# Idokorro/MiniGrid-RL

Measured on AMD Instinct MI355X. Metric: env-steps/sec at 65k parallel envs, 1/2/4/8 MI355X; % HBM roofline, higher is better.
Workload: dtype u8

## Files before the change

### minigrid-rl_amd/csrc/mgx_device.h

```cpp
#pragma once
#ifndef MGX_HOST_SIM
#include <hip/hip_runtime.h>
#else
#include "host_sim.h"
#endif
#include <stdint.h>

#include "mgx_diag.h"

namespace mgx {

constexpr uint8_t CODE_EMPTY = 0x01;
constexpr uint8_t CODE_WALL = 2 | (5 << 4);
constexpr uint8_t CODE_GOAL = 8 | (1 << 4);
constexpr uint8_t CODE_LAVA = 9;
constexpr int T_EMPTY = 1, T_WALL = 2, T_DOOR = 4, T_KEY = 5, T_BALL = 6, T_BOX = 7,
              T_GOAL = 8, T_LAVA = 9, T_OPEN = 11;
constexpr int A_LEFT = 0, A_RIGHT = 1, A_FORWARD = 2, A_PICKUP = 3, A_DROP = 4,
              A_TOGGLE = 5, A_DONE = 6;
constexpr uint8_t NONE8 = 0xFF;

__device__ __forceinline__ int cn2idx(int cn) { return (0x403512 >> (cn * 4)) & 0xF; }

__device__ __forceinline__ uint8_t mk_code(int t, int cidx, int aux) {
// ... 121 lines not shown
        x = (int)(a >> k);
        y = (int)(b >> k);
        return;
    }
    const uint64_t ma = (uint64_t)a * s, mb = (uint64_t)b * s;
    if ((uint32_t)ma < s || (uint32_t)mb < s) {
        p = p0;
        x = pcg_integers(p, 0, S);
        y = pcg_integers(p, 0, S);
        return;
    }
    x = (int)(ma >> 32);
    y = (int)(mb >> 32);
}

__device__ __forceinline__ uint32_t ss_hashmix(uint32_t v, uint32_t &hc) {
    v ^= hc; hc *= 0x931e8875u; v *= hc; v ^= v >> 16; return v;
}
__device__ __forceinline__ uint32_t ss_mix(uint32_t x, uint32_t y) {
    uint32_t r = 0xca01f9ddu * x - 0x4973f715u * y; r ^= r >> 16; return r;
}
__device__ __forceinline__ void pcg_seed(Pcg &p, uint64_t seed) {
    uint32_t e0 = (uint32_t)seed, e1 = (uint32_t)(seed >> 32);
    int nent = (seed >> 32) ? 2 : 1;
    uint32_t pool[4];
    uint32_t hc = 0x43b0d7e5u;
#pragma unroll
    for (int i = 0; i < 4; i++) pool[i] = ss_hashmix(i == 0 ? e0 : (i == 1 && nent == 2 ? e1 : 0u), hc);
#pragma unroll
    for (int s = 0; s < 4; s++)
#pragma unroll
        for (int d = 0; d < 4; d++)
            if (s != d) pool[d] = ss_mix(pool[d], ss_hashmix(pool[s], hc));
    uint32_t w[8];
    uint32_t hb = 0x8b51f9ddu;
#pragma unroll
    for (int i = 0; i < 8; i++) {
        uint32_t v = pool[i & 3];
        v ^= hb; hb *= 0x58f38dedu; v *= hb; v ^= v >> 16;
        w[i] = v;
    }
    uint64_t v0 = (uint64_t)w[0] | ((uint64_t)w[1] << 32), v1 = (uint64_t)w[2] | ((uint64_t)w[3] << 32);
    uint64_t v2 = (uint64_t)w[4] | ((uint64_t)w[5] << 32), v3 = (uint64_t)w[6] | ((uint64_t)w[7] << 32);
    p.ih = (v2 << 1) | (v3 >> 63);
    p.il = (v3 << 1) | 1ull;
    p.sh = 0; p.sl = 0;
    pcg_step(p);
    uint64_t nl = p.sl + v1;
    p.sh = p.sh + v0 + (nl < p.sl ? 1ull : 0ull);
    p.sl = nl;
    pcg_step(p);
    p.has = 0; p.uinteger = 0;
}

constexpr int MT_FIELDS = 10;
template <int NW>
__host__ __device__ constexpr int mt_wg() { return NW == 1 ? MGX_MT_WG1 : 16; }
constexpr int MT_WG_MAX = 16;
template <int NW>
__host__ __device__ constexpr int win_stride() { return 2 * mt_wg<NW>() + 2; }
__host__ __device__ constexpr int win_stride_of(int nw) { return nw == 1 ? win_stride<1>() : win_stride<2>(); }
constexpr uint64_t MT_REP = 0x041041041041041ull;
constexpr uint64_t MT_LOW60 = (1ull << 60) - 1ull;
constexpr int MAX_OBJS = 32;
constexpr int SAT_PROBE = 64;
constexpr uint32_t PCG_LOOP_LIMIT = 1u << 20;

template <int NW>
struct Bits {
    uint64_t w0, w1, w2, w3;
    __device__ __forceinline__ void clear() { w0 = w1 = w2 = w3 = 0; }
    __device__ __forceinline__ bool test(int b) const {
        const int i = b >> 6;
        uint64_t v = w0;
        if (NW > 1) v = i == 1 ? w1 : v;
        if (NW > 2) { v = i == 2 ? w2 : v; v = i == 3 ? w3 : v; }
        return (v >> (b & 63)) & 1ull;
    }
    __device__ __forceinline__ void set(int b) {
        const int i = b >> 6;
        const uint64_t m = 1ull << (b & 63);
        w0 |= i == 0 ? m : 0ull;
        if (NW > 1) w1 |= i == 1 ? m : 0ull;
        if (NW > 2) { w2 |= i == 2 ? m : 0ull; w3 |= i == 3 ? m : 0ull; }
    }
    __device__ __forceinline__ void unset(int b) {
        const int i = b >> 6;
        const uint64_t m = ~(1ull << (b & 63));
        w0 &= i == 0 ? m : ~0ull;
        if (NW > 1) w1 &= i == 1 ? m : ~0ull;
        if (NW > 2) { w2 &= i == 2 ? m : ~0ull; w3 &= i == 3 ? m : ~0ull; }
    }
};

template <>
struct Bits<4> {
    __device__ __forceinline__ void clear() {}
    __device__ __forceinline__ void set(int) {}
    __device__ __forceinline__ void unset(int) {}
};

template <int NW>
struct Gen {
    uint8_t *g;
    int S;
    Bits<NW> occ;
    Bits<NW> dn;
    const uint64_t *table;
    uint64_t rmask;
    uint64_t tlo, thi;
    uint64_t *win;
    uint64_t gbase;
    uint64_t cur, astart;
    uint64_t ga, gb, gc;
    uint64_t gi;
    int go;
    uint32_t llw;
    bool abort;
    uint32_t err;
    Pcg pcg;
    int ax, ay, adir;
    int goalx, goaly;
    bool phave;
    uint64_t prec;
    uint32_t *objs;
    int nobjs;
    uint32_t tmask;
    int problem, cfg_mission, num_objects, all_doors_open, n_obstacles;
#if MGX_GEN_STAMPS
    unsigned long long *stamps;
    uint64_t tlast;
#endif
};

#if MGX_GEN_STAMPS
#define GSTAMP(G, k)                                                                     \
    do {                                                                                 \
        const uint64_t _t = __builtin_amdgcn_s_memtime();                                \
        const unsigned long long _m = __ballot(1);                                       \
        if ((int)__lane_id() == __ffsll((long long)_m) - 1) atomicAdd(&(G).stamps[k], _t - (G).tlast); \
        (G).tlast = _t;                                                                  \
    } while (0)
#if MGX_GEN_STAMPS == 2
#define GCOUNT(G, k) do { } while (0)
#else
#define GCOUNT(G, k)                                                                     \
    do {                                                                                 \
        const unsigned long long _m = __ballot(1);                                       \
        if ((int)__lane_id() == __ffsll((long long)_m) - 1) atomicAdd(&(G).stamps[k], 1ull); \
    } while (0)
#endif
#else
#define GSTAMP(G, k) do { } while (0)
#define GCOUNT(G, k) do { } while (0)
#endif


template <int NW>
__device__ __forceinline__ void put(Gen<NW> &G, int x, int y, uint8_t code) {
    const int b = y * G.S + x;
    G.g[b] = code;
    if (code == CODE_EMPTY) G.occ.unset(b); else G.occ.set(b);
}

#ifndef MGX_HOST_SIM
typedef __attribute__((address_space(3))) uint64_t lds_u64;
#else
typedef uint64_t lds_u64;
#endif
constexpr int MT_PAD = MT_WG_MAX + 4;
template <int WG>
__device__ __noinline__ void mt_refill_cold(const uint64_t *__restrict__ table, uint64_t slot, lds_u64 *win) {
    const uint4 *src = reinterpret_cast<const uint4 *>(table + slot);
    static_assert(WG % 8 == 0 && WG <= MT_WG_MAX, "window loads go in fours of 16 B");
#pragma unroll
    for (int h = 0; h < WG / 8; h++) {
        const uint4 v0 = src[4 * h], v1 = src[4 * h + 1], v2 = src[4 * h + 2], v3 = src[4 * h + 3];
        lds_u64 *d = win + 8 * h;
        d[0] = (uint64_t)v0.x | ((uint64_t)v0.y << 32); d[1] = (uint64_t)v0.z | ((uint64_t)v0.w << 32);
        d[2] = (uint64_t)v1.x | ((uint64_t)v1.y << 32); d[3] = (uint64_t)v1.z | ((uint64_t)v1.w << 32);
        d[4] = (uint64_t)v2.x | ((uint64_t)v2.y << 32); d[5] = (uint64_t)v2.z | ((uint64_t)v2.w << 32);
        d[6] = (uint64_t)v3.x | ((uint64_t)v3.y << 32); d[7] = (uint64_t)v3.z | ((uint64_t)v3.w << 32);
    }
}
template <int NW>
__device__ __forceinline__ uint64_t win_group(Gen<NW> &G, uint64_t g) {
    constexpr int MT_WG = mt_wg<NW>();
    uint64_t off = g - G.gbase;
    if (off >= MT_WG) {
        GCOUNT(G, 23);
        if (g < G.tlo || g + MT_WG > G.thi) G.err |= 1u;
        mt_refill_cold<MT_WG>(G.table, g & G.rmask, (lds_u64 *)G.win);
        G.gbase = g;
        off = 0;
    }
    return G.win[off];
}
__device__ __forceinline__ uint64_t div10(uint64_t v) { return __umul64hi(v, 0xCCCCCCCCCCCCCCCDull) >> 3; }
template <int NW>
__device__ __forceinline__ void mt_sync(Gen<NW> &G) {
    const uint64_t g = div10(G.cur);
    G.go = (int)(G.cur - g * MT_FIELDS);
    G.gi = g;
    G.ga = win_group(G, g);
    G.gb = win_group(G, g + 1);
    G.gc = win_group(G, g + 2);
}
struct RbConst {
    uint64_t c1;
    uint32_t sh;
};
__device__ __forceinline__ RbConst rb_const(uint32_t n) {
    const uint32_t sh = 5u - (uint32_t)(32 - __clz(n));
    return RbConst{(uint64_t)(32u + (n << sh) - 1u) * MT_REP, sh};
}
template <int NW>
__device__ __forceinline__ int randbelow_c(Gen<NW> &G, const RbConst K);
template <int NW>
__device__ __forceinline__ int randbelow(Gen<NW> &G, uint32_t n) {
    GCOUNT(G, 24);
    if (n >= 32u) { G.err |= 8u; return 0; }
    return randbelow_c(G, rb_const(n));
}
template <int NW>
__device__ __forceinline__ int randbelow_c(Gen<NW> &G, const RbConst K) {
    const uint64_t c1 = K.c1;
    const uint32_t sh = K.sh;
    for (;;) {
        GCOUNT(G, 21);
        const int o6 = (int)__umul24((uint32_t)G.go, 6u);
        const uint64_t f = ((G.ga >> o6) | (G.gb << (60 - o6))) & MT_LOW60;
        const uint64_t acc = (c1 - f) & (32ull * MT_REP);
        const uint32_t left = G.llw - (uint32_t)(G.cur - G.astart);
        const int j = acc ? (int)(((uint32_t)__ffsll((long long)acc) - 1u - 5u) * 171u >> 10) : MT_FIELDS;
        int m = j < MT_FIELDS ? j + 1 : MT_FIELDS;
        if ((uint32_t)m > left) {
            G.cur = G.astart + G.llw;
            G.abort = true;
            return 0;
        }
        const int r = (int)(((f >> (6 * (j < MT_FIELDS ? j : 0))) & 31u) >> sh);
        G.cur += (uint64_t)m;
        G.go += m;
        if (G.go >= MT_FIELDS) {
            G.go -= MT_FIELDS;
            G.ga = G.gb;
            G.gb = G.gc;
            G.gi++;
            G.gc = win_group(G, G.gi + 2);
        }
        if (j < MT_FIELDS) return r;
    }
}
template <class GT>
__device__ __forceinline__ void mt_advance(GT &G, int m) {
    G.cur += (uint64_t)m;
    G.go += m;
    if (G.go >= MT_FIELDS) {
        G.go -= MT_FIELDS;
        G.ga = G.gb;
        G.gb = G.gc;
        G.gi++;
        G.gc = win_group(G, G.gi + 2);
    }
}
template <class GT>
__device__ __forceinline__ uint64_t randbelow_seq(GT &G, uint64_t prog, int cnt) {
    constexpr uint64_t GM = 32ull * MT_REP;
    uint64_t res = 0;
    int i = 0;
#pragma unroll 1
    while (i < cnt) {
        GCOUNT(G, 21);
        const int o6 = (int)__umul24((uint32_t)G.go, 6u);
        const uint64_t f = ((G.ga >> o6) | (G.gb << (60 - o6))) & MT_LOW60;
        uint64_t avail = GM;
        int used = MT_FIELDS;
#pragma unroll 1
        while (i < cnt) {
            const RbConst K = rb_const((uint32_t)(prog >> (5 * i)) & 31u);
            const uint64_t acc = (K.c1 - f) & avail;
            if (!acc) { used = MT_FIELDS; break; }
            const int b = __ffsll((long long)acc) - 1;
            res |= (uint64_t)((((uint32_t)(f >> (b - 5))) & 31u) >> K.sh) << (5 * i);
            avail &= ~((2ull << b) - 1ull);
            used = (int)((uint32_t)(b + 1) * 171u >> 10);
            i++;
        }
        const uint32_t left = G.llw - (uint32_t)(G.cur - G.astart);
        if ((uint32_t)used > left) {
            G.cur = G.astart + G.llw;
            G.abort = true;
            return res;
        }
        mt_advance(G, used);
    }
    return res;
}
template <int NW, typename Bad, typename Sat>
__device__ __forceinline__ void draw_cell(Gen<NW> &G, const RbConst KX, const RbConst KY, int x0, int y0, int &x, int &y,
                                          Bad bad, Sat sat ,
                                          bool has_c, const RbConst KC, int &choice) {
    constexpr uint64_t GM = 32ull * MT_REP;
    int rej = 0;
    bool need_c = has_c;
#pragma unroll 1
    for (;;) {
        GCOUNT(G, 21);
        const int o6 = (int)__umul24((uint32_t)G.go, 6u);
        const uint64_t f = ((G.ga >> o6) | (G.gb << (60 - o6))) & MT_LOW60;
        uint64_t avail = GM;
        int used = 0;
        if (need_c) {
            const uint64_t acc = (KC.c1 - f) & GM;
            if (!acc) {
                const uint32_t left = G.llw - (uint32_t)(G.cur - G.astart);
                if ((uint32_t)MT_FIELDS > left) {
                    G.cur = G.astart + G.llw;
                    G.abort = true;
                    return;
                }
                mt_advance(G, MT_FIELDS);
                continue;
            }
            const int b = __ffsll((long long)acc) - 1;
            choice = (int)((((uint32_t)(f >> (b - 5))) & 31u) >> KC.sh);
            avail &= ~((2ull << b) - 1ull);
            used = (int)((uint32_t)(b + 1) * 171u >> 10);
            need_c = false;
        }
        const uint64_t accx = (KX.c1 - f) & GM, accy = (KY.c1 - f) & GM;
        bool ok = false;
#pragma unroll 1
        for (;;) {
            const uint64_t cx = accx & avail;
            if (!cx) break;
            const int bx = __ffsll((long long)cx) - 1;
            const uint64_t cy = accy & avail & ~((2ull << bx) - 1ull);
            if (!cy) break;
            const int by = __ffsll((long long)cy) - 1;
            x = x0 + (int)(((uint32_t)(f >> (bx - 5)) & 31u) >> KX.sh);
            y = y0 + (int)(((uint32_t)(f >> (by - 5)) & 31u) >> KY.sh);
            used = (int)((uint32_t)(by + 1) * 171u >> 10);
            avail &= ~((2ull << by) - 1ull);
            if (!bad(x, y)) { ok = true; break; }
            if (++rej == SAT_PROBE && !sat()) { live_lock(G); return; }
        }
        const uint32_t left = G.llw - (uint32_t)(G.cur - G.astart);
        if ((uint32_t)used > left) {
            G.cur = G.astart + G.llw;
            G.abort = true;
            return;
        }
        mt_advance(G, used);
        if (ok) return;
        x = x0 + randbelow_c(G, KX);
        y = y0 + randbelow_c(G, KY);
        if (G.abort) return;
        if (!bad(x, y)) return;
        if (++rej == SAT_PROBE && !sat()) { live_lock(G); return; }
    }
}

template <int NW>
__device__ __forceinline__ int randint(Gen<NW> &G, int a, int b) { return a + randbelow(G, (uint32_t)(b - a + 1)); }
template <int NW>
__device__ __forceinline__ bool choice_bool(Gen<NW> &G) { return randbelow(G, 2) == 0; }

template <int NW>
__device__ __forceinline__ bool next2door(const Gen<NW> &G, int x, int y) {
    if constexpr (NW == 4) {
        return is_door(G.g[y * G.S + x - 1]) || is_door(G.g[y * G.S + x + 1]) ||
               is_door(G.g[(y - 1) * G.S + x]) || is_door(G.g[(y + 1) * G.S + x]);
    } else {
        return G.dn.test(y * G.S + x);
    }
}
template <int NW>
__device__ __forceinline__ bool occupied(const Gen<NW> &G, int b) {
    if constexpr (NW == 4) return G.g[b] != CODE_EMPTY;
    else return G.occ.test(b);
}

constexpr uint32_t OBJ_KEYFLAG = 1u << 24;
template <int NW>
__device__ __forceinline__ void add_obj(Gen<NW> &G, int t, int cname, int x, int y, uint32_t flags = 0) {
    const bool full = G.nobjs >= MAX_OBJS;
    G.err |= full ? 8u : 0u;
    G.tmask |= full ? 0u : 1u << t;
    const bool first_goal = !full && t == T_GOAL && G.goalx < 0;
    G.goalx = first_goal ? x : G.goalx;
    G.goaly = first_goal ? y : G.goaly;
    if (!full)
        G.objs[G.nobjs++] = (uint32_t)t | ((uint32_t)(cname & 15) << 4) | ((uint32_t)x << 8) | ((uint32_t)y << 16) | flags;
}

template <int NW>
__device__ __forceinline__ void draw_free_cell(Gen<NW> &G, int &px, int &py) {
    for (uint32_t it = 0;; ++it) {
        GCOUNT(G, 22);
        if (it > PCG_LOOP_LIMIT) { G.err |= 4u; px = 1; py = 1; return; }
        int x, y;
        pcg_cell(G.pcg, G.S, x, y);
        if (occupied(G, y * G.S + x)) continue;
        if (x == G.ax && y == G.ay) continue;
        px = x; py = y;
        return;
    }
}
template <int NW>
__device__ __forceinline__ void place_agent(Gen<NW> &G) {
    G.ax = -1; G.ay = -1;
    int x, y;
    draw_free_cell(G, x, y);
    G.ax = x; G.ay = y;
    G.adir = pcg_integers(G.pcg, 0, 4);
}

__device__ __forceinline__ int nth_set_bit(uint32_t m, int r) {
    int pos = 0, c;
    c = __popc(m & 0xFFFFu); if (r >= c) { r -= c; m >>= 16; pos += 16; }
    c = __popc(m & 0xFFu);   if (r >= c) { r -= c; m >>= 8;  pos += 8; }
    c = __popc(m & 0xFu);    if (r >= c) { r -= c; m >>= 4;  pos += 4; }
    c = __popc(m & 0x3u);    if (r >= c) { r -= c; m >>= 2;  pos += 2; }
    c = (int)(m & 1u);       if (r >= c) { pos += 1; }
    return pos;
}
template <int NW>
__device__ __forceinline__ int mask_choice(Gen<NW> &G, uint32_t m) {
    return nth_set_bit(m, randbelow(G, (uint32_t)__popc(m)));
}

template <int NW>
__device__ __forceinline__ void live_lock(Gen<NW> &G) {
    G.cur = G.astart + G.llw;
    G.abort = true;
}

template <int NW>
__device__ __forceinline__ void place_key(Gen<NW> &G, int x0, int x1, int y0, int y1, int gx, int gy, bool chk_agent,
                                          int ox, int oy, int cname, bool kib, int *kx, int *ky) {
    int x, y, rej = 0;
    for (;;) {
        x = randint(G, x0, x1);
        y = randint(G, y0, y1);
        if (G.abort) return;
        const bool bad = (x == gx && y == gy) || (chk_agent && x == G.ax && y == G.ay) || (x == ox && y == oy) ||
                         next2door(G, x, y);
        if (!bad) break;
        if (++rej == SAT_PROBE) {
            bool sat = false;
            for (int xx = x0; xx <= x1 && !sat; xx++)
                for (int yy = y0; yy <= y1 && !sat; yy++)
                    sat = !((xx == gx && yy == gy) || (chk_agent && xx == G.ax && yy == G.ay) ||
                            (xx == ox && yy == oy) || next2door(G, xx, yy));
            if (!sat) { live_lock(G); return; }
        }
    }
    const int cidx = cn2idx(cname);
    if (kib) { put(G, x, y, mk_code(T_BOX, cidx, 1)); add_obj(G, T_BOX, cname, x, y, OBJ_KEYFLAG); }
    else { put(G, x, y, mk_code(T_KEY, cidx, 0)); add_obj(G, T_KEY, cname, x, y, OBJ_KEYFLAG); }
    if (kx) { *kx = x; *ky = y; }
}

template <int NW>
__device__ __forceinline__ void place_objects(Gen<NW> &G, uint32_t &oc, const int *types, int n, int x0, int x1,
                                              int y0, int y1) {
    for (int k = 0; k < n; k++) {
        if (oc == 0) { G.err |= 8u; return; }
        const int b = mask_choice(G, oc);
        if (G.abort) return;
        oc &= ~(1u << b);
        const int t = types[b / 6], cname = b % 6;
        int x, y, rej = 0;
        for (;;) {
            x = randint(G, x0, x1);
            y = randint(G, y0, y1);
            if (G.abort) return;
            const bool bad = occupied(G, y * G.S + x) || (x == G.ax && y == G.ay) || next2door(G, x, y);
            if (!bad) break;
            if (++rej == SAT_PROBE) {
                bool sat = false;
                for (int xx = x0; xx <= x1 && !sat; xx++)
                    for (int yy = y0; yy <= y1 && !sat; yy++)
                        sat = !(occupied(G, yy * G.S + xx) || (xx == G.ax && yy == G.ay) || next2door(G, xx, yy));
                if (!sat) { live_lock(G); return; }
            }
        }
        put(G, x, y, mk_code(t, cn2idx(cname), 0));
        add_obj(G, t, cname, x, y);
    }
}

__device__ __forceinline__ int door_code(int cname, bool locked, bool open) {
    return open ? mk_code(T_OPEN, cn2idx(cname), 0) : mk_code(T_DOOR, cn2idx(cname), locked ? 1 : 0);
}

template <int NW>
__device__ __forceinline__ void put_door(Gen<NW> &G, int x, int y, uint8_t code) {
    put(G, x, y, code);
    const int S = G.S, b = y * S + x;
    if (x > 0) G.dn.set(b - 1);
    if (x < S - 1) G.dn.set(b + 1);
    if (y > 0) G.dn.set(b - S);
    if (y < S - 1) G.dn.set(b + S);
}

template <int NW>
__device__ __forceinline__ uint32_t bits_row(const Bits<NW> &B, int y, int S) {
    const int b = y * S;
    uint64_t v = b < 64 ? (B.w0 >> b) : 0ull;
    if (NW > 1) {
        if (b >= 64) v = B.w1 >> (b - 64);
// ... 67 lines not shown
    } else if (r == 1) {
        if (ar == 1) { kA = VL; kB = HL; } else if (ar == 3) kA = HL; else if (ar == 0) kA = VL;
    } else if (r == 2) {
        if (ar == 2) { kA = VU; kB = HR; } else if (ar == 3) kA = VU; else if (ar == 0) kA = HR;
    } else {
        if (ar == 3) { kA = VL; kB = HR; } else if (ar == 1) kA = HR; else if (ar == 2) kA = VL;
    }
}

__device__ const int MULTI_TYPES[3] = {T_KEY, T_BALL, T_BOX};

struct Prefix {
    int nr, rc;
    uint32_t dinfo;
    uint32_t dpos;
    uint32_t dopen;
};
template <class GT>
__device__ __forceinline__ void prefix_draws(GT &G, int S, bool draw_cmd, bool ado, Prefix &P) {
    const uint64_t r = randbelow_seq(G, draw_cmd ? (4ull | (3ull << 5)) : 3ull, draw_cmd ? 2 : 1);
    P.rc = draw_cmd ? (int)(r & 31) : 0;
    P.nr = 2 + (int)((draw_cmd ? r >> 5 : r) & 31);
    P.dinfo = P.dpos = P.dopen = 0;
    if (G.abort || (MGX_GEN_SKIP & 8)) return;
    const int nr = P.nr, mid = S / 2, ndoors = nr == 2 ? 1 : nr;
    uint64_t prog = 0;
    int cnt = 0;
#pragma unroll 1
    for (int d = 0; d < ndoors; d++) {
        prog |= (uint64_t)(6 - d) << (5 * cnt++);
        if (!ado) prog |= 2ull << (5 * cnt++);
        prog |= 2ull << (5 * cnt++);
    }
    const uint64_t dr = randbelow_seq(G, prog, cnt);
    if (G.abort) return;
    uint32_t dc = 0x3Fu;
#pragma unroll 1
    for (int d = 0, k = 0; d < ndoors; d++) {
        const int col = nth_set_bit(dc, (int)(dr >> (5 * k++)) & 31);
        dc &= ~(1u << col);
        const bool lk = ado ? false : ((dr >> (5 * k++)) & 31) == 0;
        const bool kib = ((dr >> (5 * k++)) & 31) == 0;
        P.dinfo |= (uint32_t)(col | (lk << 3) | (kib << 4)) << (8 * d);
    }
    prog = 0;
    cnt = 0;
#pragma unroll 1
    for (int d = 0; d < ndoors; d++) {
        bool horiz; int lo, hi;
        door_geom(nr, d, mid, S, horiz, lo, hi);
        prog |= (uint64_t)(hi - lo + 1) << (5 * cnt++);
        if (ado) prog |= 2ull << (5 * cnt++);
    }
    const uint64_t pr = randbelow_seq(G, prog, (MGX_GEN_SKIP & 2) ? 0 : cnt);
    if (G.abort) return;
#pragma unroll 1
    for (int d = 0, k = 0; d < ((MGX_GEN_SKIP & 2) ? 0 : ndoors); d++) {
        P.dpos |= (uint32_t)((pr >> (5 * k++)) & 15) << (4 * d);
        if (ado) P.dopen |= (uint32_t)(((pr >> (5 * k++)) & 31) == 0) << d;
    }
}
constexpr int PFX_LOOK = 320;
__host__ __device__ __forceinline__ uint64_t pfx_pack(const Prefix &P, uint32_t adv, uint32_t tag) {
    uint64_t r = (uint64_t)(adv & 0xFF) | ((uint64_t)(tag & 0xFF) << 8) | ((uint64_t)(P.nr - 2) << 16) |
                 ((uint64_t)(P.rc & 3) << 18);
    for (int d = 0; d < 4; d++)
        r |= (uint64_t)(((P.dinfo >> (8 * d)) & 31) | (((P.dpos >> (4 * d)) & 15) << 5) | (((P.dopen >> d) & 1) << 9))
             << (20 + 10 * d);
    return r;
}
__host__ __device__ __forceinline__ void pfx_unpack(uint64_t r, Prefix &P) {
    P.nr = 2 + (int)((r >> 16) & 3);
    P.rc = (int)((r >> 18) & 3);
    P.dinfo = P.dpos = P.dopen = 0;
    for (int d = 0; d < 4; d++) {
        const uint32_t f = (uint32_t)(r >> (20 + 10 * d)) & 0x3FFu;
        P.dinfo |= (f & 31u) << (8 * d);
        P.dpos |= ((f >> 5) & 15u) << (4 * d);
        P.dopen |= ((f >> 9) & 1u) << d;
    }
}
constexpr int MT_SB_WORDS = 3120;
constexpr int MT_SB_GROUPS = MT_SB_WORDS / MT_FIELDS;
constexpr int MT_SLIDE_MAX_SB = 64;
__host__ __device__ __forceinline__ int mt_slide_superblocks(unsigned long long hi, unsigned long long need_lo,
                                                             unsigned long long want_hi,
                                                             unsigned long long ring_groups) {
    int nsb = 0;
    while (nsb < MT_SLIDE_MAX_SB && hi + (unsigned long long)nsb * MT_SB_GROUPS < want_hi &&
           hi + (unsigned long long)(nsb + 1) * MT_SB_GROUPS <= need_lo + ring_groups)
        nsb++;
    return nsb;
}
struct PfxWindow {
    unsigned long long zero_lo, rec_lo, rec_hi;
    unsigned long long next_done;
    unsigned long long strides;
};
__host__ __device__ __forceinline__ PfxWindow pfx_window(unsigned long long rec_done, unsigned long long hi,
                                                         unsigned long long ring_words, unsigned long long threads,
                                                         unsigned long long look) {
    const unsigned long long top = hi * (unsigned long long)MT_FIELDS;
    const unsigned long long held = top > ring_words ? top - ring_words : 0ull;
    PfxWindow w;
    w.rec_hi = top > look ? top - look : 0ull;
    w.rec_lo = rec_done > held ? rec_done : held;
    if (w.rec_hi < w.rec_lo) w.rec_hi = w.rec_lo;
    w.zero_lo = w.rec_lo;
    if (rec_done < held) {
        const unsigned long long kept = w.rec_hi > ring_words ? w.rec_hi - ring_words : 0ull;
        w.zero_lo = rec_done > kept ? rec_done : kept;
    }
    w.next_done = w.rec_hi;
    w.strides = (w.rec_hi - w.rec_lo + threads - 1) / threads;
    return w;
}

template <int NW>
__device__ __forceinline__ void gen_rooms(Gen<NW> &G, const Prefix &P) {
    const int S = G.S, mid = S / 2, nr = P.nr;
    if (MGX_GEN_SKIP & 8) { G.ax = 1; G.ay = 1; put(G, S - 2, S - 2, CODE_GOAL); add_obj(G, T_GOAL, 15, S - 2, S - 2); return; }
    for (int i = 1; i < S - 1; i++) put(G, mid, i, CODE_WALL);
    if (nr == 3) for (int i = 1; i < mid; i++) put(G, i, mid, CODE_WALL);
    if (nr == 4) for (int i = 1; i < S - 1; i++) put(G, i, mid, CODE_WALL);
    const int ndoors = nr == 2 ? 1 : nr;
    const bool ado = G.all_doors_open;
    const uint32_t dinfo = P.dinfo;
    uint32_t oc = 0x3FFFFu;
#pragma unroll 1
    for (int d = 0; d < ndoors; d++) {
        const uint32_t di = dinfo >> (8 * d);
        const int col = di & 7;
        if ((di >> 3) & 1) { oc &= ~(1u << col); if ((di >> 4) & 1) oc &= ~(1u << (12 + col)); }
    }
    GSTAMP(G, 11);
#pragma unroll 1
    for (int d = 0; d < ((MGX_GEN_SKIP & 2) ? 0 : ndoors); d++) {
        bool horiz; int lo, hi;
        door_geom(nr, d, mid, S, horiz, lo, hi);
        const int v = lo + (int)((P.dpos >> (4 * d)) & 15);
        const int x = horiz ? v : mid, y = horiz ? mid : v;
        const uint32_t di = dinfo >> (8 * d);
        const bool open = ado && ((P.dopen >> d) & 1);
        put_door(G, x, y, (uint8_t)door_code(di & 7, (di >> 3) & 1, open));
        add_obj(G, T_DOOR, di & 7, x, y);
    }
    GSTAMP(G, 12);
    if (G.abort) return;
    int gx = 1, gy = 1;
    if (MGX_GEN_SKIP & 4) {
        gx = 1; gy = 1; put(G, gx, gy, CODE_GOAL); add_obj(G, T_GOAL, 15, gx, gy); G.ax = S - 2; G.ay = S - 2;
    } else {
        bool agent = false;
#pragma unroll 1
        for (uint32_t it = 0;; ++it) {
            GCOUNT(G, 22);
            if (it > 2 * PCG_LOOP_LIMIT) { G.err |= 4u; G.ax = 1; G.ay = 1; break; }
            int x, y;
            pcg_cell(G.pcg, S, x, y);
            if (occupied(G, y * S + x)) continue;
            if (agent) { G.ax = x; G.ay = y; break; }
            if (next2door(G, x, y)) continue;
            gx = x; gy = y;
            put(G, gx, gy, CODE_GOAL);
            add_obj(G, T_GOAL, 15, gx, gy);
            agent = true;
        }
        G.adir = pcg_integers(G.pcg, 0, 4);
    }
    GSTAMP(G, 13);
    const int gr = room_of(nr, gx, gy, mid), ar = room_of(nr, G.ax, G.ay, mid);
    const int n_left = G.num_objects / 2, n_right = G.num_objects - n_left;
    int c0, c1, c2, c3;
    if (nr == 2) { c0 = n_left; c1 = n_right; c2 = c3 = 0; }
    else if (nr == 3) { c0 = n_left / 2; c1 = n_left - c0; c2 = n_right; c3 = 0; }
    else { c0 = n_left / 2; c1 = n_left - c0; c2 = n_right / 2; c3 = n_right - c2; }
    uint32_t keymask = 0;
    uint32_t npack = 0;
    uint32_t kspec = 0;
#pragma unroll
    for (int r = 0; r < 4; r++) {
        int kA, kB;
        bool chk;
        key_spec(nr, r, ar, kA, kB, chk);
        kspec |= (uint32_t)(kA & 3) << (4 * r) | (uint32_t)(kB & 3) << (4 * r + 2) | (uint32_t)chk << (16 + r);
        const bool a = r < nr && kA >= 0 && ((dinfo >> (8 * kA + 3)) & 1);
        const bool b = r < nr && kB >= 0 && ((dinfo >> (8 * kB + 3)) & 1);
        keymask |= (uint32_t)a << (2 * r) | (uint32_t)b << (2 * r + 1);
        const int ndec = (int)a + (int)b + (int)(gr == r);
        int n;
        if (r == 0) { c0 -= ndec; n = c0; }
        else if (r == 1) { c1 -= ndec; n = (nr == 2) ? c1 : c0; }
        else if (r == 2) { c2 -= ndec; n = c2; }
        else { c3 -= ndec; n = c3; }
        npack |= (uint32_t)(n > 0 ? n : 0) << (8 * r);
    }
    uint64_t reps = 0;
    if (NW == 1)
        for (int i = 0; i < S; i++) reps |= 1ull << (i * S);
    uint64_t todo = 0;
#pragma unroll
    for (int rr = 0; rr < 4; rr++)
        todo |= (uint64_t)(((keymask >> (2 * rr)) & 3u) | ((((1u << ((npack >> (8 * rr)) & 0xFF)) - 1u) & 0x3FFFu) << 2))
                << (16 * rr);
    if (MGX_GEN_SKIP & 1) return;
    int kx = -1, ky = -1;
#pragma unroll 1
    while (todo) {
        GCOUNT(G, 20);
        GSTAMP(G, 19);
        GSTAMP(G, 16);
        const int slot = (int)__builtin_ctzll(todo);
        const int r = slot >> 4, phase = min(slot & 15, 2);
        int x0, x1, y0, y1;
        room_rect(nr, r, mid, S, x0, x1, y0, y1);
        const bool is_key = phase < 2;
        int cname, ot = T_KEY, ox = -1, oy = -1;
        bool chk = false, kib = false;
        if (is_key) {
            chk = (kspec >> (16 + r)) & 1;
            const uint32_t di = dinfo >> (8 * ((kspec >> (4 * r + 2 * phase)) & 3));
            cname = di & 7;
            kib = (di >> 4) & 1;
            if (phase == 1 && ((keymask >> (2 * r)) & 1)) { ox = kx; oy = ky; }
        } else {
            if (oc == 0) { G.err |= 8u; break; }
        }
        const bool has_c = !is_key && !(MGX_GEN_SKIP & 32);
        const RbConst kc_ = rb_const(is_key ? 1u : (uint32_t)__popc(oc));
        int choice = 0;
        const int ex0 = is_key ? gx : G.ax, ey0 = is_key ? gy : G.ay;
        const int ex1 = (is_key && !chk) ? -1 : G.ax, ey1 = (is_key && !chk) ? -1 : G.ay;
        const RbConst kx_ = rb_const((uint32_t)(x1 - x0 + 1)), ky_ = rb_const((uint32_t)(y1 - y0 + 1));
        int x, y;
        GSTAMP(G, 17);
        if constexpr (NW <= 2) {
            Bits<NW> bad = G.dn;
            if (!is_key) { bad.w0 |= G.occ.w0; if (NW > 1) bad.w1 |= G.occ.w1; }
            bad.set(ey0 * S + ex0);
            if (ex1 >= 0) bad.set(ey1 * S + ex1);
            if (ox >= 0) bad.set(oy * S + ox);
            bool sat;
            if constexpr (NW == 1) {
                const uint64_t rows = reps & (((1ull << ((y1 + 1) * S)) - 1ull) & ~((1ull << (y0 * S)) - 1ull));
                sat = ((rows * (uint64_t)(((1u << (x1 - x0 + 1)) - 1u) << x0)) & ~bad.w0) != 0;
            } else {
                sat = rect_has_free(G, x0, x1, y0, y1, !is_key, ex0, ey0, ex1, ey1, ox, oy);
            }
            if (!sat) {
                live_lock(G);
                return;
            }
            draw_cell(G, kx_, ky_, x0, y0, x, y, [&](int cx, int cy) { return bad.test(cy * S + cx); },
                      [] { return true; }, has_c, kc_, choice);
            if (G.abort) return;
        } else {
            const auto bad = [&](int cx, int cy) {
                return (cx == ex0 && cy == ey0) || (cx == ex1 && cy == ey1) || (cx == ox && cy == oy) ||
                       (!is_key && occupied(G, cy * S + cx)) || next2door(G, cx, cy);
            };
            draw_cell(G, kx_, ky_, x0, y0, x, y, bad, [&] {
                for (int xx = x0; xx <= x1; xx++)
                    for (int yy = y0; yy <= y1; yy++)
                        if (!bad(xx, yy)) return true;
                return false;
            }, has_c, kc_, choice);
            if (G.abort) return;
        }
        if (!is_key) {
            const int b = (MGX_GEN_SKIP & 32) ? __ffs(oc) - 1 : nth_set_bit(oc, choice);
            oc &= ~(1u << b);
            ot = MULTI_TYPES[b / 6];
            cname = b % 6;
        }
        GSTAMP(G, 18);
        const int cidx = cn2idx(cname);
        const int t = is_key ? (kib ? T_BOX : T_KEY) : ot;
        put(G, x, y, mk_code(t, cidx, (is_key && kib) ? 1 : 0));
        add_obj(G, t, cname, x, y, is_key ? OBJ_KEYFLAG : 0u);
        if (phase == 0) { kx = x; ky = y; }
        todo &= todo - 1;
    }
    GSTAMP(G, 14);
}

template <int NW>
__device__ __forceinline__ int gen_multi(Gen<NW> &G) {
    const bool draw_cmd = G.cfg_mission < 0;
    Prefix P;
    if (G.phave) {
        pfx_unpack(G.prec, P);
    } else {
#if MGX_GEN_PREFIX2
        { const uint64_t c0_ = G.cur; prefix_draws(G, G.S, draw_cmd, G.all_doors_open != 0, P); G.cur = c0_; G.abort = false; mt_sync(G); }
#endif
        prefix_draws(G, G.S, draw_cmd, G.all_doors_open != 0, P);
        if (G.abort) return 0;
    }
    const int cmd = draw_cmd ? (P.rc == 3 ? 5 : P.rc) : G.cfg_mission;
    GSTAMP(G, 10);
    gen_rooms(G, P);
    return cmd;
}

__device__ const int GTO_T[4] = {T_KEY, T_BALL, T_BOX, T_DOOR};
__device__ const int GTG_T[4] = {T_BOX, T_DOOR, T_KEY, T_BALL};
__device__ const int OPN_T[2] = {T_BOX, T_DOOR};
__device__ const int PKP_T[3] = {T_KEY, T_BOX, T_BALL};

template <int NW, bool EXT>
__device__ __forceinline__ int gen_single(Gen<NW> &G) {
    const int *types;
    int ntypes, cmd;
    bool goal = false;
    const bool full = EXT && G.problem == 1;
    if constexpr (EXT) {
        switch (G.problem) {
            case 1: types = GTO_T; ntypes = 4; cmd = -1; goal = true; break;
            case 2: types = GTO_T; ntypes = 4; cmd = 0; break;
// ... 251 lines not shown
```

### minigrid-rl_amd/csrc/mgx_engine.hip

```cpp
#include <hip/hip_runtime.h>

#include <algorithm>
#include <cmath>
#include <cstdio>
#include <cstdlib>
#include <cstring>
#include <new>
#include <string>
#include <vector>

#include "../../include/mgx.h"
#include "mgx_diag.h"
#include "mgx_device.h"

using namespace mgx;

namespace {

constexpr int BLOCK_ENVS = 64;
typedef uint16_t rpos_t;
constexpr int MGX_MAX_RING = 4096;
constexpr uint32_t NO_POP = 0xFFFFFFFFu;
constexpr int MGX_NCOUNTERS = 32;
constexpr int BLOCK_THREADS = 256;
// ... 1504 lines not shown
    Q.rmask = p.mt_mask;
    Q.cur = Q.astart = pos;
    const uint64_t g = div10(pos);
    Q.go = (int)(pos - g * MT_FIELDS);
    Q.gi = g;
    Q.ga = win_group(Q, g);
    Q.gb = win_group(Q, g + 1);
    Q.gc = win_group(Q, g + 2);
    Q.llw = p.llw;
    Q.err = 0;
    Q.abort = false;
    Prefix P;
    prefix_draws(Q, p.S, p.cfg_mission < 0, p.all_doors_open != 0, P);
    const uint64_t adv = Q.cur - pos;
    if (Q.abort || adv == 0 || adv > 255) return 0;
    return pfx_pack(P, (uint32_t)adv, pfx_tag(pos, p.mt_shift));
#endif
}
__global__ __launch_bounds__(256) void mgx_prefix_kernel(KParams p, uint64_t lo, uint64_t hi) {
    for (uint64_t pos = lo + (uint64_t)blockIdx.x * blockDim.x + threadIdx.x; pos < hi;
         pos += (uint64_t)gridDim.x * blockDim.x)
        p.pfx[pfx_index(pos, p.mt_mask)] = pfx_compute(p, pos);
}

template <int NW, bool EXT, bool MULTI, int SC = 0, int EPW = 64>
__device__ __forceinline__ void refill_body(const KParams &p) {
    extern __shared__ __align__(16) uint8_t smem[];
    const int tid = threadIdx.x;
    const int64_t e = tid < EPW ? (int64_t)blockIdx.x * EPW + tid : INT64_MAX;
    uint8_t *s_grid = smem;
    uint8_t *s_scr = smem + ((64 * p.GSL + 15) & ~15);
    unsigned long long maxcur = 0;
    uint32_t err = 0;
    __shared__ unsigned int s_pfx[2];
    if (tid == 0) s_pfx[0] = s_pfx[1] = 0u;
    if (p.refill_prio == 1) __builtin_amdgcn_s_setprio(1);
    else if (p.refill_prio == 2) __builtin_amdgcn_s_setprio(2);
    else if (p.refill_prio == 3) __builtin_amdgcn_s_setprio(3);
    __shared__ unsigned long long s_t0;
    if (p.clk.slots && tid == 0) s_t0 = clk_now();
#if MGX_REFILL_CLOCK
    const unsigned long long rc0 = __builtin_amdgcn_s_memtime();
    int rc_iters = 0;
#endif
    rpos_t tail = 0;
    int level = 0, cons = 0;
    if (e < p.n) {
        const rpos_t head = *reinterpret_cast<volatile const rpos_t *>(p.ring_head + e);
        tail = p.ring_tail[e];
        level = (int)(rpos_t)(tail - head);
        cons = (int)(rpos_t)(head - p.ring_seen[e]);
        p.ring_seen[e] = head;
    }
    const int space = p.D - level, need = 2 * p.K - level;
    int cap = p.cap;
    if (cap > 0 && !p.initial_fill) {
        int sum = e < p.n ? cons : 0, cnt = e < p.n ? 1 : 0;
        for (int off = 32; off > 0; off >>= 1) {
            sum += __shfl_xor(sum, off);
            cnt += __shfl_xor(cnt, off);
        }
        cnt = max(cnt, 1);
        cap = (sum + cnt - 1) / cnt;
        const int rc = p.mtc->round_cap;
        if (rc > 0) cap = min(cap, rc);
    }
    int nfree = 0, nmin = 0;
    if (e < p.n) {
        nfree = p.initial_fill ? space : max(need, p.cap < 0 ? space : min(cap, space));
        nfree = min(nfree, space);
        nmin = max(need, 0);
    }
    const bool producer = nfree > 0;
    if (__ballot(producer)) {
        Gen<NW> G;
        load_gen(G, p, e, s_grid + tid * p.GSL, s_scr, tid);
        if (SC > 0) G.S = SC;
        int livelocks = 0;
        if (producer) {
            load_rng(G, p, e);
            livelocks = (int)(p.aux[e].y >> 1);
        }
        uint32_t *const stg = G.objs;
        uint64_t nrec = 0;
        if (producer && p.pfx) nrec = p.pfx[pfx_index(G.cur, p.mt_mask)];
        unsigned long long act;
        while ((act = __ballot(nfree > 0)) != 0) {
#if MGX_REFILL_CLOCK
            rc_iters += nfree > 0;
#endif
            const bool hit = nfree > 0 && p.pfx && (nrec & 0xFFu) &&
                             ((uint32_t)(nrec >> 8) & 0xFFu) == pfx_tag(G.cur, p.mt_shift);
            if (p.pfx) {
                const int nh = __popcll(__ballot(hit));
                if (tid == 0) {
                    s_pfx[0] += (unsigned int)__popcll(act);
                    s_pfx[1] += (unsigned int)nh;
                }
            }
            bool wrote = false;
            uint32_t slot = 0;
            if (nfree > 0) {
                ResetOut R;
                G.astart = G.cur;
                G.abort = false;
                G.phave = hit;
                G.prec = nrec;
                if (G.phave) G.cur += nrec & 0xFFu;
                mt_sync(G);
                gen_attempt<NW, EXT, MULTI>(G, R);
                if (p.pfx) nrec = p.pfx[pfx_index(G.cur, p.mt_mask)];
                if (G.nobjs > p.obj_cap) G.err |= 8u;
                if (G.abort && ++livelocks <= 100000) {
                    if (nfree > nmin) nfree--;
                } else {
                    if (G.abort) G.err |= 4u;
                    R.livelocks = livelocks;
                    livelocks = 0;
                    nfree--;
                    nmin--;
                    slot = (uint32_t)e * (uint32_t)p.D + (tail & (p.D - 1));
                    const uint4 h = pack_hdr(G, R);
                    uint4 rs[2];
                    rng_snapshot(G, rs);
                    stg[0] = h.x; stg[1] = h.y; stg[2] = h.z; stg[3] = h.w;
                    stg[4] = rs[0].x; stg[5] = rs[0].y; stg[6] = rs[0].z; stg[7] = rs[0].w;
                    stg[8] = rs[1].x; stg[9] = rs[1].y; stg[10] = rs[1].z; stg[11] = rs[1].w;
                    if (EXT && p.has_move) p.ring_range[slot] = R.range;
                    tail++;
                    wrote = true;
                }
            }
            const unsigned long long wm = __ballot(wrote);
            __builtin_amdgcn_fence(__ATOMIC_RELEASE, "wavefront");
            __builtin_amdgcn_fence(__ATOMIC_ACQUIRE, "wavefront");
            const int REC = SC > 0 ? ((((SC * SC + 15) & ~15) + 48 + 63) & ~63) : p.REC;
            const int P = REC >> 4, GQ = (SC > 0 ? ((SC * SC + 15) & ~15) : p.GS) >> 4;
            const uint8_t *objs0 = reinterpret_cast<const uint8_t *>(stg) - tid * (p.obj_stride * 4);
            for (int q = tid; q < 64 * P; q += 64) {
                const int src = q / P, j = q - src * P;
                const uint32_t ss = (uint32_t)__shfl((int)slot, src);
                if (!((wm >> src) & 1ull)) continue;
                const uint32_t *w = j < GQ ? reinterpret_cast<const uint32_t *>(s_grid + src * p.GSL + 16 * j)
                                           : reinterpret_cast<const uint32_t *>(objs0 + src * (p.obj_stride * 4) +
                                                                                 16 * (j - GQ));
                uint4 v = make_uint4(0u, 0u, 0u, 0u);
                if (j < GQ + 3) v = make_uint4(w[0], w[1], w[2], w[3]);
                st16<MGX_NT_REC != 0>(reinterpret_cast<uint4 *>(p.ring_rec + (size_t)ss * (size_t)REC) + j, v);
            }
            __builtin_amdgcn_fence(__ATOMIC_RELEASE, "wavefront");
            __builtin_amdgcn_fence(__ATOMIC_ACQUIRE, "wavefront");
        }
        if (producer) {
            store_rng(G, p, e, (uint32_t)livelocks);
            p.ring_tail[e] = tail;
            maxcur = G.cur;
            err = G.err;
        }
    }
    for (int off = 32; off > 0; off >>= 1) {
        unsigned long long o = __shfl_down(maxcur, off);
        maxcur = o > maxcur ? o : maxcur;
        err |= __shfl_down(err, off);
#if MGX_REFILL_CLOCK
        rc_iters = max(rc_iters, __shfl_down(rc_iters, off));
#endif
    }
#if MGX_REFILL_CLOCK
    if (tid == 0) {
        atomicAdd(&p.counters[26], __builtin_amdgcn_s_memtime() - rc0);
        atomicAdd(&p.counters[27], (unsigned long long)rc_iters);
        atomicAdd(&p.counters[28], 1ull);
        atomicAdd(&p.counters[8 + min(rc_iters, 15)], 1ull);
        atomicMax(&p.counters[29], __builtin_amdgcn_s_memtime() - rc0);
    }
#endif
    int csum = e < p.n ? cons : 0;
    for (int off = 32; off > 0; off >>= 1) csum += __shfl_xor(csum, off);
    if (tid == 0) {
        ulonglong4 b = p.blk[2 * p.nblk + blockIdx.x];
        b.w = b.w > maxcur ? b.w : maxcur;
        b.x = (unsigned long long)csum;
        b.y += (unsigned long long)s_pfx[0];
        b.z += (unsigned long long)s_pfx[1];
        p.blk[2 * p.nblk + blockIdx.x] = b;
        if (err) atomicOr(p.err, err);
        if (p.clk.slots) clk_record(p.clk, CLK_REFILL, s_t0);
    }
}

template <int NW, bool EXT>
__global__ __launch_bounds__(64) void mgx_refill_kernel(KParams p) { refill_body<NW, EXT, false>(p); }
template <>
__global__ __launch_bounds__(64, 3) void mgx_refill_kernel<1, false>(KParams p) {
    refill_body<1, false, false>(p);
}
template <int NW>
__global__ __launch_bounds__(64) void mgx_refill_multi_kernel(KParams p) { refill_body<NW, false, true>(p); }
template <>
__global__ __launch_bounds__(64, 3) void mgx_refill_multi_kernel<1>(KParams p) {
    refill_body<1, false, true>(p);
}
template <int EPW>
__global__ __launch_bounds__(64, 3) void mgx_refill_s8_kernel(KParams p) { refill_body<1, false, true, 8, EPW>(p); }

template <int NW, bool EXT>
__global__ __launch_bounds__(64) void mgx_scene_kernel(KParams p, int64_t e, uint32_t *__restrict__ rec) {
    extern __shared__ __align__(16) uint8_t smem[];
    if (threadIdx.x != 0) return;
    uint8_t *s_grid = smem;
    uint8_t *s_scr = smem + ((64 * p.GSL + 15) & ~15);
    Gen<NW> G;
    load_gen(G, p, e, s_grid, s_scr, 0);
    const uint4 c0 = p.start_rng[2 * e], c1 = p.start_rng[2 * e + 1], inc = p.pcg[2 * e + 1];
    G.pcg.sh = ((uint64_t)c0.x << 32) | c0.y;
    G.pcg.sl = ((uint64_t)c0.z << 32) | c0.w;
    G.pcg.ih = ((uint64_t)inc.x << 32) | inc.y;
    G.pcg.il = ((uint64_t)inc.z << 32) | inc.w;
    G.pcg.uinteger = c1.x;
    G.pcg.has = c1.y & 1u;
    G.cur = (uint64_t)c1.z | ((uint64_t)c1.w << 32);
    G.gbase = ~0ull >> 1;
    ResetOut R;
    reset_env<NW, EXT>(G, R);
    rec[0] = (uint32_t)G.nobjs;
    rec[1] = (uint32_t)G.ax | ((uint32_t)G.ay << 8) | ((uint32_t)G.adir << 16);
    rec[2] = (uint32_t)R.mission_id | ((uint32_t)R.tx << 8) | ((uint32_t)R.ty << 16) | ((uint32_t)R.ta << 24);
    rec[3] = (uint32_t)R.livelocks;
    rec[4] = G.err;
    for (int k = 0; k < MAX_OBJS; k++) rec[8 + k] = k < G.nobjs ? G.objs[k] : 0u;
    for (int k = 0; k < p.S * p.S; k++) reinterpret_cast<uint8_t *>(rec + 8 + MAX_OBJS)[k] = G.g[k];
}

__device__ __forceinline__ uint32_t mt_mix(uint32_t a, uint32_t b, uint32_t x) {
    const uint32_t y = (a & 0x80000000u) | (b & 0x7fffffffu);
    return x ^ (y >> 1) ^ ((y & 1u) ? 0x9908b0dfu : 0u);
}
__device__ __forceinline__ void mt_twist_block(uint32_t *s, int tid) {
    uint32_t v = 0;
    if (tid < 227) v = mt_mix(s[tid], s[tid + 1], s[tid + 397]);
    __syncthreads();
    if (tid < 227) s[tid] = v;
    __syncthreads();
    const int i = 227 + tid;
    if (tid < 227) v = mt_mix(s[i], s[i + 1], s[i - 227]);
    __syncthreads();
    if (tid < 227) s[i] = v;
    __syncthreads();
    const int k = 454 + tid;
    if (tid < 170) v = mt_mix(s[k], s[k == 623 ? 0 : k + 1], s[k - 227]);
    __syncthreads();
    if (tid < 170) s[k] = v;
    __syncthreads();
}
__device__ __forceinline__ uint32_t mt_temper(uint32_t y) {
    y ^= y >> 11;
    y ^= (y << 7) & 0x9d2c5680u;
    y ^= (y << 15) & 0xefc60000u;
    return y ^ (y >> 18);
}

__global__ __launch_bounds__(SLIDE_THREADS) void mgx_mt_slide_kernel(KParams p) {
    __shared__ uint32_t s_st[624];
    __shared__ uint8_t s_f[MT_SB_WORDS];
    __shared__ unsigned long long s_red[SLIDE_THREADS / 64], s_red2[SLIDE_THREADS / 64];
    __shared__ unsigned long long s_hi;
    __shared__ int s_nsb;
    const int tid = threadIdx.x;
    MtCtl *c = p.mtc;
    __shared__ unsigned long long s_t0;
    if (p.clk.slots && tid == 0) s_t0 = clk_now();
    unsigned long long mn = ~0ull, mx = 0;
    const int64_t e0 = (int64_t)blockIdx.x * SLIDE_ENVS;
    constexpr int EPT = SLIDE_ENVS / SLIDE_THREADS;
    rpos_t tl[EPT];
    unsigned long long cu[EPT], pc[EPT];
#pragma unroll
    for (int k = 0; k < EPT; k++) {
        const int64_t e = e0 + k * SLIDE_THREADS + tid;
        const bool in = e < p.n;
        const int64_t ec = in ? e : 0;
        tl[k] = p.D > 0 ? p.ring_tail[ec] : (rpos_t)0;
        const uint2 cr = reinterpret_cast<const uint2 *>(p.cur_rng + 2 * ec + 1)[1];
        const uint2 ax = reinterpret_cast<const uint2 *>(p.aux + ec)[1];
        cu[k] = in ? ((unsigned long long)cr.x | ((unsigned long long)cr.y << 32)) : ~0ull;
        pc[k] = in ? ((unsigned long long)ax.x | ((unsigned long long)ax.y << 32)) : 0ull;
    }
#pragma unroll
    for (int k = 0; k < EPT; k++) {
        const int64_t e = e0 + k * SLIDE_THREADS + tid;
        if (e < p.n) {
            if (p.D > 0) p.ring_pubn[e] = tl[k];
            unsigned long long v = cu[k];
            if (p.start_rng) {
                const uint4 sr = p.start_rng[2 * e + 1];
                const unsigned long long u = (unsigned long long)sr.z | ((unsigned long long)sr.w << 32);
                v = u < v ? u : v;
            }
            mn = v < mn ? v : mn;
            mx = pc[k] > mx ? pc[k] : mx;
        }
    }
    unsigned long long rec_next = 0;
    if (p.pfx) {
        const unsigned long long T = (unsigned long long)gridDim.x * SLIDE_THREADS;
        const PfxWindow w = pfx_window(c->rec_done, c->hi, (p.mt_mask + 1) * (unsigned long long)MT_FIELDS, T,
                                       (unsigned long long)PFX_LOOK);
        const unsigned long long t0 = (unsigned long long)blockIdx.x * SLIDE_THREADS + tid;
// ... 1506 lines not shown
```

Measured before the change: 2.474 billion.

## Branchless draw_cell field scan and fused goal/agent placement mask

Rewrites the rejection-sampling cell draw to compress the 60-bit acceptance mask into a 10-bit field mask with a multiply trick. It then selects fields with ctz and select operations instead of ffsll and branches, inlines the MT window advance, and retries by consuming a full group rather than falling back to randbelow_c. Goal/agent placement for small grids merges the occupancy and door-neighbor bitmasks into one test and defers the goal write until after the agent is placed. The producer's store index is also recomputed from the block and lane to steer register allocation. This changes the RNG consumption pattern, which risks altering sampled layouts relative to the reference.

```diff
diff --git a/minigrid-rl_amd/csrc/mgx_device.h b/minigrid-rl_amd/csrc/mgx_device.h
--- a/minigrid-rl_amd/csrc/mgx_device.h
+++ b/minigrid-rl_amd/csrc/mgx_device.h
@@ -297,7 +297,11 @@
 #endif
 #else
 #define GSTAMP(G, k) do { } while (0)
+#ifdef MGX_GCOUNT_HOOK
+#define GCOUNT(G, k) MGX_GCOUNT_HOOK(k)
+#else
 #define GCOUNT(G, k) do { } while (0)
+#endif
 #endif
 
 
@@ -442,68 +446,70 @@
     }
     return res;
 }
+__device__ __forceinline__ uint32_t guard10(uint64_t acc) {
+    constexpr uint32_t K = (1u << 20) | (1u << 15) | (1u << 10) | (1u << 5) | 1u;
+    const uint32_t lo = (uint32_t)acc >> 5, hi = (uint32_t)(acc >> 32) >> 3;
+    return (((lo * K) >> 20) & 31u) | ((((hi * K) >> 20) & 31u) << 5);
+}
 template <int NW, typename Bad, typename Sat>
 __device__ __forceinline__ void draw_cell(Gen<NW> &G, const RbConst KX, const RbConst KY, int x0, int y0, int &x, int &y,
                                           Bad bad, Sat sat ,
                                           bool has_c, const RbConst KC, int &choice) {
     constexpr uint64_t GM = 32ull * MT_REP;
     int rej = 0;
-    bool need_c = has_c;
+    bool need_c = has_c, have_x = false;
+    uint32_t xv = 0;
 #pragma unroll 1
     for (;;) {
+        GCOUNT(G, 27);
         GCOUNT(G, 21);
         const int o6 = (int)__umul24((uint32_t)G.go, 6u);
         const uint64_t f = ((G.ga >> o6) | (G.gb << (60 - o6))) & MT_LOW60;
-        uint64_t avail = GM;
-        int used = 0;
+        uint32_t avail = 0x3FFu;
         if (need_c) {
-            const uint64_t acc = (KC.c1 - f) & GM;
-            if (!acc) {
-                const uint32_t left = G.llw - (uint32_t)(G.cur - G.astart);
-                if ((uint32_t)MT_FIELDS > left) {
-                    G.cur = G.astart + G.llw;
-                    G.abort = true;
-                    return;
-                }
-                mt_advance(G, MT_FIELDS);
-                continue;
-            }
-            const int b = __ffsll((long long)acc) - 1;
-            choice = (int)((((uint32_t)(f >> (b - 5))) & 31u) >> KC.sh);
-            avail &= ~((2ull << b) - 1ull);
-            used = (int)((uint32_t)(b + 1) * 171u >> 10);
-            need_c = false;
-        }
-        const uint64_t accx = (KX.c1 - f) & GM, accy = (KY.c1 - f) & GM;
-        bool ok = false;
+            const uint32_t mc = guard10((KC.c1 - f) & GM);
+            const uint32_t j = (uint32_t)__builtin_ctz(mc | 0x400u);
+            choice = mc ? (int)((((uint32_t)(f >> (6u * j))) & 31u) >> KC.sh) : choice;
+            avail &= ~1u << j;
+            need_c = mc == 0u;
+        }
+        const uint32_t mx = guard10((KX.c1 - f) & GM), my = guard10((KY.c1 - f) & GM);
+        bool ok;
+        uint32_t jy;
 #pragma unroll 1
         for (;;) {
-            const uint64_t cx = accx & avail;
-            if (!cx) break;
-            const int bx = __ffsll((long long)cx) - 1;
-            const uint64_t cy = accy & avail & ~((2ull << bx) - 1ull);
-            if (!cy) break;
-            const int by = __ffsll((long long)cy) - 1;
-            x = x0 + (int)(((uint32_t)(f >> (bx - 5)) & 31u) >> KX.sh);
-            y = y0 + (int)(((uint32_t)(f >> (by - 5)) & 31u) >> KY.sh);
-            used = (int)((uint32_t)(by + 1) * 171u >> 10);
-            avail &= ~((2ull << by) - 1ull);
-            if (!bad(x, y)) { ok = true; break; }
+            GCOUNT(G, 25);
+            const uint32_t cx = mx & avail;
+            const uint32_t jx = (uint32_t)__builtin_ctz(cx | 0x400u);
+            const uint32_t xn = (((uint32_t)(f >> (6u * jx))) & 31u) >> KX.sh;
+            const uint32_t av = have_x ? avail : avail & (~1u << jx);
+            xv = have_x ? xv : xn;
+            const uint32_t cy = my & av;
+            jy = (uint32_t)__builtin_ctz(cy | 0x400u);
+            x = x0 + (int)xv;
+            y = y0 + (int)((((uint32_t)(f >> (6u * jy))) & 31u) >> KY.sh);
+            avail = av & (~1u << jy);
+            have_x = cy == 0u && (have_x || cx != 0u);
+            ok = cy != 0u && !bad(x, y);
+            if (ok || cy == 0u) break;
             if (++rej == SAT_PROBE && !sat()) { live_lock(G); return; }
         }
+        const int used = ok ? (int)jy + 1 : MT_FIELDS;
         const uint32_t left = G.llw - (uint32_t)(G.cur - G.astart);
         if ((uint32_t)used > left) {
             G.cur = G.astart + G.llw;
             G.abort = true;
             return;
         }
-        mt_advance(G, used);
+        G.cur += (uint64_t)used;
+        G.go += used;
+        const bool rot = G.go >= MT_FIELDS;
+        G.go -= rot ? MT_FIELDS : 0;
+        G.ga = rot ? G.gb : G.ga;
+        G.gb = rot ? G.gc : G.gb;
+        G.gi += rot ? 1ull : 0ull;
+        G.gc = win_group(G, G.gi + 2);
         if (ok) return;
-        x = x0 + randbelow_c(G, KX);
-        y = y0 + randbelow_c(G, KY);
-        if (G.abort) return;
-        if (!bad(x, y)) return;
-        if (++rej == SAT_PROBE && !sat()) { live_lock(G); return; }
     }
 }
 
@@ -877,19 +883,42 @@
         gx = 1; gy = 1; put(G, gx, gy, CODE_GOAL); add_obj(G, T_GOAL, 15, gx, gy); G.ax = S - 2; G.ay = S - 2;
     } else {
         bool agent = false;
+        int gcell = -1;
+        if constexpr (NW <= 2) {
 #pragma unroll 1
-        for (uint32_t it = 0;; ++it) {
-            GCOUNT(G, 22);
-            if (it > 2 * PCG_LOOP_LIMIT) { G.err |= 4u; G.ax = 1; G.ay = 1; break; }
-            int x, y;
-            pcg_cell(G.pcg, S, x, y);
-            if (occupied(G, y * S + x)) continue;
-            if (agent) { G.ax = x; G.ay = y; break; }
-            if (next2door(G, x, y)) continue;
-            gx = x; gy = y;
+            for (uint32_t it = 0;; ++it) {
+                GCOUNT(G, 22);
+                if (it > 2 * PCG_LOOP_LIMIT) { G.err |= 4u; G.ax = 1; G.ay = 1; break; }
+                int x, y;
+                pcg_cell(G.pcg, S, x, y);
+                const int b = y * S + x;
+                Bits<NW> rejm = G.occ;
+                rejm.w0 |= agent ? 0ull : G.dn.w0;
+                if (NW > 1) rejm.w1 |= agent ? 0ull : G.dn.w1;
+                if (rejm.test(b)) continue;
+                if (agent) { G.ax = x; G.ay = y; break; }
+                gx = x; gy = y; gcell = b;
+                G.occ.set(b);
+                agent = true;
+            }
+        } else {
+#pragma unroll 1
+            for (uint32_t it = 0;; ++it) {
+                GCOUNT(G, 22);
+                if (it > 2 * PCG_LOOP_LIMIT) { G.err |= 4u; G.ax = 1; G.ay = 1; break; }
+                int x, y;
+                pcg_cell(G.pcg, S, x, y);
+                const int b = y * S + x;
+                if (occupied(G, b) || b == gcell) continue;
+                if (agent) { G.ax = x; G.ay = y; break; }
+                if (next2door(G, x, y)) continue;
+                gx = x; gy = y; gcell = b;
+                agent = true;
+            }
+        }
+        if (gcell >= 0) {
             put(G, gx, gy, CODE_GOAL);
             add_obj(G, T_GOAL, 15, gx, gy);
-            agent = true;
         }
         G.adir = pcg_integers(G.pcg, 0, 4);
     }
diff --git a/minigrid-rl_amd/csrc/mgx_engine.hip b/minigrid-rl_amd/csrc/mgx_engine.hip
--- a/minigrid-rl_amd/csrc/mgx_engine.hip
+++ b/minigrid-rl_amd/csrc/mgx_engine.hip
@@ -1680,8 +1680,11 @@
             __builtin_amdgcn_fence(__ATOMIC_ACQUIRE, "wavefront");
         }
         if (producer) {
-            store_rng(G, p, e, (uint32_t)livelocks);
-            p.ring_tail[e] = tail;
+            int lane = tid;
+            asm volatile("" : "+v"(lane));
+            const int64_t e2 = (int64_t)blockIdx.x * EPW + lane;
+            store_rng(G, p, e2, (uint32_t)livelocks);
+            p.ring_tail[e2] = tail;
             maxcur = G.cur;
             err = G.err;
         }
```

Result: faster. 2.557 billion, median of 6 (+3.4%).
